# hrdkjain/GenIcoNet

Measured on AMD Instinct MI355X. Metric: meshes/sec training throughput, ico2ico I5 batch=36, higher is better.
Workload: dtype f32; 1 GPU; ico2ico AE training, I5, batch 36 per GPU (BASELINE configs[1]); per_gpu_batch=36, global_batch=36, subdivisions=5, parallelism=dp1

## Files before the change

geniconet_amd/csrc/icn_api.cpp:

```cpp
#include <hip/hip_runtime.h>

#include <algorithm>
#include <cmath>
#include <cstdio>
#include <cstdlib>
#include <cstring>
#include <map>
#include <mutex>
#include <stdexcept>
#include <string>
#include <tuple>
#include <vector>

#include "../../include/icn_ext.h"
#include "../../include/icn_curvature.h"
#include "../../include/icn_gauss.h"
#include "../../include/icn_measure.h"
#include "icn_geometry.h"
#include "icn_launch.h"
#include "icn_streamk.h"

namespace {

thread_local std::string g_err;
// ... 1 lines not shown
int fail(const std::string& msg) {
    g_err = msg;
    return -1;
}

#define ICN_HIP(expr)                                                                       \
    do {                                                                                    \
        hipError_t e_ = (expr);                                                             \
        if (e_ != hipSuccess) throw std::runtime_error(std::string(#expr) + ": " + hipGetErrorString(e_)); \
    } while (0)

template <typename R, typename F>
R returns(F&& body) {
    try {
        return body();
    } catch (const std::exception& e) {
        return (R)fail(e.what());
    }
}
template <typename R, typename F>
R returns_or_zero(F&& body) {
    try {
        return body();
    } catch (const std::exception&) {
        return 0;
    }
}
template <typename F>
int guarded(F&& body) {
    return returns<int>([&] { body(); return 0; });
}
template <typename F>
int launched(F&& body) {
    return returns<int>([&] { body(); ICN_HIP(hipGetLastError()); return 0; });
}

template <typename T>
long copy_out(T* dst, size_t cap, const std::vector<T>& v) {
    if (dst) std::memcpy(dst, v.data(), std::min(cap, v.size()) * sizeof(T));
    return (long)v.size();
}

thread_local bool g_dry_run = false;
thread_local size_t g_dry_elems = 0;

template <typename T>
T* upload(const std::vector<T>& v) {
    T* d = nullptr;
    if (v.empty()) return d;
    if (g_dry_run) {
        g_dry_elems += v.size();
        return d;
    }
    ICN_HIP(hipMalloc(reinterpret_cast<void**>(&d), v.size() * sizeof(T)));
    ICN_HIP(hipMemcpy(d, v.data(), v.size() * sizeof(T), hipMemcpyHostToDevice));
    return d;
}

struct DevDma {
    int32_t* code = nullptr;
    int32_t* slots = nullptr;
    int n_slots = 0, E = 1;
};
DevDma upload_dma(const std::vector<int32_t>& idx, int E, int P) {
    icn::DmaTable h;
    icn::build_dma_table(idx, E, P, h);
    DevDma d;
    d.code = upload(h.code);
    d.slots = upload(h.slots);
    d.n_slots = h.n_slots;
    d.E = E;
    return d;
}
struct ConvTables {
    int Pin = 0, Pout = 0, n_in = 0, n_out = 0, E = 1;
    int32_t* fwd = nullptr;
    int32_t* bwd = nullptr;
    int32_t* bwd1 = nullptr;
    int nv = 0, nvp = 0;
    int32_t* vidx = nullptr;
    int32_t* vorder = nullptr;
    uint32_t* vmask32 = nullptr;
    int32_t* vq = nullptr;
    int32_t* perm = nullptr;
    int32_t* bwd_perm = nullptr;
    uint32_t* mask32 = nullptr;
    std::vector<uint32_t> mask32_h;
    int key = 0;
    DevDma d_fwd, d_bwd, d_bwd1, d_virt, d_bwdp;
    int32_t* w7_rows = nullptr;
    uint16_t* w7_pos = nullptr;
    int w7_U = 0;
};
struct UpTables {
    int Pc = 0, Pf = 0, Wf = 0, Wb = 0;
    int32_t *idx_f = nullptr, *idx_b = nullptr;
    float *coef_f = nullptr, *coef_b = nullptr;
};

struct UpconvDev {
    int Pc = 0, Pf = 0, n_slots = 0, E = 1, nseg = 0;
    int seg_cnt[icn::UPCONV_MAX_SEG] = {}, seg_off[icn::UPCONV_MAX_SEG] = {};
    uint32_t seg_mask[icn::UPCONV_MAX_SEG] = {};
    int32_t *pix = nullptr, *code = nullptr, *slot_idx = nullptr;
    float *alpha = nullptr, *slot_coef = nullptr;
};

struct EllSplitDev {
    int W = 0, n_ovf = 0, W_ovf = 0;
    int32_t *idx = nullptr, *ovf_rows = nullptr, *ovf_idx = nullptr;
    float *coef = nullptr, *ovf_coef = nullptr;
};
EllSplitDev upload_ell_split(const icn::Ell& e, int W_main) {
    EllSplitDev d;
    const int W = e.width;
    d.W = W_main;
    d.W_ovf = std::max(W - W_main, 0);
    std::vector<int32_t> idx((size_t)e.rows * W_main, icn::IDX_ZERO), ovf_rows, ovf_idx;
    std::vector<float> coef((size_t)e.rows * W_main, 0.f), ovf_coef;
    for (int r = 0; r < e.rows; ++r) {
        for (int k = 0; k < std::min(W, W_main); ++k) {
            idx[(size_t)r * W_main + k] = e.idx[(size_t)r * W + k];
            coef[(size_t)r * W_main + k] = e.coef[(size_t)r * W + k];
        }
        if (W > W_main && e.idx[(size_t)r * W + W_main] != icn::IDX_ZERO) {
            ovf_rows.push_back(r);
            for (int k = W_main; k < W; ++k) {
                ovf_idx.push_back(e.idx[(size_t)r * W + k]);
                ovf_coef.push_back(e.coef[(size_t)r * W + k]);
            }
        }
    }
    d.n_ovf = (int)ovf_rows.size();
    d.idx = upload(idx);
    d.coef = upload(coef);
    d.ovf_rows = upload(ovf_rows);
    d.ovf_idx = upload(ovf_idx);
    d.ovf_coef = upload(ovf_coef);
    return d;
}

struct PatchHost { std::vector<int32_t> prow; std::vector<uint16_t> plocal; int npatch = 0, umax = 0, gridW = 0; };
bool build_patches(const std::vector<int32_t>& idx, int width_in, int width, int H, int W, int ph, int pw, PatchHost& out) {
    out = PatchHost{};
    if (H % ph != 0 || W % pw != 0 || (long)H * W * width_in != (long)idx.size()) return false;
    const int pr_n = H / ph, pc_n = W / pw;
    out.npatch = pr_n * pc_n;
    out.gridW = W;
    out.plocal.assign((size_t)H * W * width, 0xFFFFu);
    std::vector<std::vector<int32_t>> lists(out.npatch);
    for (int p = 0; p < out.npatch; ++p) {
        std::vector<int32_t>& u = lists[p];
        for (int i = 0; i < ph; ++i)
            for (int j = 0; j < pw; ++j) {
                const size_t r = (size_t)((p / pc_n) * ph + i) * W + (p % pc_n) * pw + j;
                for (int k = 0; k < width; ++k) {
                    const int32_t v = idx[r * width_in + k];
                    if (v >= 0) u.push_back(v);
                }
            }
        std::sort(u.begin(), u.end());
        u.erase(std::unique(u.begin(), u.end()), u.end());
        out.umax = std::max(out.umax, (int)u.size());
    }
    out.umax = (out.umax + 31) / 32 * 32;
    if (out.umax == 0 || out.umax >= 0xFFFF) return false;
// ... 7 lines not shown
                for (int k = 0; k < width; ++k) {
                    const int32_t v = idx[r * width_in + k];
                    if (v >= 0) out.plocal[r * width + k] = (uint16_t)(std::lower_bound(u.begin(), u.end(), v) - u.begin());
                }
            }
    }
    return true;
}
struct PatchDev { int32_t* prow = nullptr; uint16_t* plocal = nullptr; int npatch = 0, umax = 0, gridW = 0; };
PatchDev upload_patches(const PatchHost& h) {
    PatchDev d;
    if (getenv("ICN_VERBOSE")) fprintf(stderr, "icn: patch table: %d patches, %d rows per list, grid width %d\n", h.npatch, h.umax, h.gridW);
    d.prow = upload(h.prow);
    d.plocal = upload(h.plocal);
    d.npatch = h.npatch; d.umax = h.umax; d.gridW = h.gridW;
    return d;
}

struct UpconvBwdDev {
    int Pc = 0, Pf = 0;
    PatchDev sc_patch, ga_patch;
    EllSplitDev gather, scatter;
    int32_t* iota = nullptr;
    int32_t* px_srcs = nullptr;
    int32_t* px_cls = nullptr;
    float* cls_coef = nullptr;
    int n_cls = 0;
};

std::mutex g_mu;
std::map<std::tuple<int, int, int>, UpconvDev> g_upconv;
std::map<std::tuple<int, int, int>, UpconvBwdDev> g_upconv_bwd;
std::map<std::tuple<int, int, int, int>, ConvTables> g_conv;
std::map<std::tuple<int, int, int>, UpTables> g_up;

static int wgrad7_union_rows(int stride) {
    if (stride != 1) return 112;
    static const int u1 = [] {
        const char* e = getenv("ICN_W7_U");
        return e ? atoi(e) : 64;
    }();
    if (u1 != 56 && u1 != 64)
        throw std::invalid_argument("icn: ICN_W7_U must be 56 or 64 (the instantiations of k_wgrad7 at stride 1), got " + std::to_string(u1));
    return u1;
}

ConvTables make_conv_tables(int r_in, int stride, int mode) {
    ConvTables t;
    t.n_in = 1 << r_in;
    t.n_out = t.n_in / stride;
    t.Pin = icn::pixels(r_in);
    t.Pout = 10 * t.n_out * t.n_out;
    std::vector<int32_t> fwd, bwd, perm;
    std::vector<uint8_t> mask;
    icn::build_conv_fwd(r_in, stride, mode, fwd);
    t.E = icn::build_conv_bwd(r_in, stride, mode, bwd);
    t.fwd = upload(fwd);
    t.bwd = upload(bwd);
    t.d_fwd = upload_dma(fwd, 1, t.Pout);
    t.d_bwd = upload_dma(bwd, t.E, t.Pin);
    {
        icn::DmaTable h;
        icn::build_dma_table(fwd, 1, t.Pout, h);
        icn::Wg7Table w7;
        if (icn::build_wgrad7(h, t.Pout, wgrad7_union_rows(stride), w7)) {
            t.w7_rows = upload(w7.urow);
            t.w7_pos = upload(w7.upos);
            t.w7_U = w7.U;
        }
    }
    std::vector<int32_t> primary;
    icn::VirtualRows vr;
    icn::split_conv_bwd(r_in, stride, bwd, t.E, primary, vr);
    t.bwd1 = upload(primary);
    t.d_bwd1 = upload_dma(primary, 1, t.Pin);
    t.nv = vr.nv;
    if (vr.nv > 0) {
        std::vector<int32_t> order, vidx_o;
        std::vector<uint8_t> vmask;
        icn::build_virtual_order(vr, t.nvp, order, vidx_o, vmask);
        t.vidx = upload(vidx_o);
        t.vorder = upload(order);
        t.vmask32 = upload(std::vector<uint32_t>(vmask.begin(), vmask.end()));
        t.d_virt = upload_dma(vidx_o, 1, t.nvp);
        t.vq = upload(vr.vq);
    }
    if (stride == 2) {
        icn::build_bwd_row_order(r_in, stride, bwd, t.E, perm, mask);
        t.perm = upload(perm);
        t.mask32_h.assign(mask.begin(), mask.end());
        t.mask32 = upload(t.mask32_h);
        t.key = 1 + ((r_in << 8) | (stride << 4) | mode);
        std::vector<int32_t> bwd_p(bwd.size());
        for (int te = 0; te < icn::NTAPS * t.E; ++te)
            for (int k = 0; k < t.Pin; ++k) bwd_p[(size_t)te * t.Pin + k] = bwd[(size_t)te * t.Pin + perm[k]];
        t.bwd_perm = upload(bwd_p);
        t.d_bwdp = upload_dma(bwd_p, t.E, t.Pin);
    }
    return t;
}
const ConvTables& conv_tables(int r_in, int stride, int mode) {
    int dev = 0;
    ICN_HIP(hipGetDevice(&dev));
    std::lock_guard<std::mutex> lk(g_mu);
    auto key = std::make_tuple(dev, r_in, stride, mode);
    auto it = g_conv.find(key);
    if (it != g_conv.end()) return it->second;
    return g_conv.emplace(key, make_conv_tables(r_in, stride, mode)).first->second;
}

std::map<std::pair<int, int>, int32_t*> g_vf;

const int32_t* vertex_faces(int r) {
    int dev = 0;
    ICN_HIP(hipGetDevice(&dev));
    std::lock_guard<std::mutex> lk(g_mu);
    auto key = std::make_pair(dev, r);
    auto it = g_vf.find(key);
    if (it != g_vf.end()) return it->second;
    std::vector<int32_t> vf;
    icn::build_vertex_faces(r, vf);
    return g_vf.emplace(key, upload(vf)).first->second;
}

std::map<std::pair<int, int>, int32_t*> g_vs;

const int32_t* vertex_stencils(int r) {
    int dev = 0;
    ICN_HIP(hipGetDevice(&dev));
    std::lock_guard<std::mutex> lk(g_mu);
    auto key = std::make_pair(dev, r);
    auto it = g_vs.find(key);
    if (it != g_vs.end()) return it->second;
    std::vector<int32_t> vs;
    icn::build_vertex_stencils(r, vs);
    return g_vs.emplace(key, upload(vs)).first->second;
}

UpTables make_up_tables(int r_in, int mode) {
    icn::Ell f, b;
    icn::build_upsample(r_in, mode, f, b);
    UpTables t;
    t.Pc = b.rows;
    t.Pf = f.rows;
    t.Wf = f.width;
    t.Wb = b.width;
    t.idx_f = upload(f.idx);
    t.coef_f = upload(f.coef);
    t.idx_b = upload(b.idx);
    t.coef_b = upload(b.coef);
    return t;
}
const UpTables& up_tables(int r_in, int mode) {
    int dev = 0;
    ICN_HIP(hipGetDevice(&dev));
    std::lock_guard<std::mutex> lk(g_mu);
    auto key = std::make_tuple(dev, r_in, mode);
    auto it = g_up.find(key);
    if (it != g_up.end()) return it->second;
    return g_up.emplace(key, make_up_tables(r_in, mode)).first->second;
}

UpconvDev make_upconv_tables(int r_in, int mode) {
    icn::UpconvTable h;
    icn::build_upconv_fwd(r_in, mode, h);
    UpconvDev d;
    d.Pc = h.Pc; d.Pf = h.Pf; d.n_slots = h.n_slots; d.E = h.E; d.nseg = h.nseg;
    for (int i = 0; i < h.nseg; ++i) { d.seg_cnt[i] = h.seg_cnt[i]; d.seg_off[i] = h.seg_off[i]; d.seg_mask[i] = h.seg_mask[i]; }
// ... 227 lines not shown
    a.wt = bn ? static_cast<const float*>(p.packed_b3) : wreg;
}
size_t conv_ws_bytes(int op, int B, int Cin, int C0, int C1, int r_in, int stride) {
    const int C = C0 + C1, n_out = (1 << r_in) / stride, M = B * 10 * n_out * n_out;
    const size_t wbytes = wpack_bytes((size_t)7 * Cin * C);
    switch (op) {
        case ICN_OP_CONV_FWD:
            if (!icn::gather_gemm_supported(Cin, C)) return 0;
            return wbytes + (C1 ? align256((size_t)C * sizeof(float)) : 0) +
                   align256((size_t)B * table_counts(r_in, stride).slots_fwd * Cin * sizeof(float)) + sk_ws_bytes();
        case ICN_OP_CONV_BWD_DATA: {
            if (!icn::gather_gemm_supported(C, Cin)) return 0;
            const TableCounts c = table_counts(r_in, stride);
            return wbytes + align256((size_t)B * c.nv * Cin * sizeof(float)) +
                   (C1 ? 2 : 1) * align256((size_t)B * c.slots_bwd * C0 * sizeof(float)) + sk_ws_bytes();
        }
        case ICN_OP_CONV_BWD_WEIGHT:
            return wgrad_partial_bytes(M, Cin, C, C0) + wgrad_bias_partial_bytes(M, Cin, C, C0) +
                   align256((size_t)B * table_counts(r_in, stride).slots_fwd * Cin * sizeof(float));
        default: return 0;
    }
}

char* at(void* ws, size_t off) { return static_cast<char*>(ws) + off; }

void conv_fwd_impl(const float* x, const float* w0, const float* b0, const float* w1, const float* b1, float* y0, float* y1, int B,
                   int Cin, int C0, int C1, int r_in, int stride, const ConvTables& t, void* ws, hipStream_t s) {
    const int C = C0 + C1;
    const size_t wbytes = wpack_bytes((size_t)7 * Cin * C);
    float* wf = static_cast<float*>(ws);
    float* bias_cat = (w1 && b0) ? reinterpret_cast<float*>(at(ws, wbytes)) : nullptr;
    const size_t side_off = wbytes + (w1 ? align256((size_t)C * sizeof(float)) : 0);
    float* side = reinterpret_cast<float*>(at(ws, side_off));
    int* sk_flag = reinterpret_cast<int*>(at(ws, side_off + align256((size_t)B * table_counts(r_in, stride).slots_fwd * Cin * sizeof(float))));
    float* sk_part = reinterpret_cast<float*>(reinterpret_cast<char*>(sk_flag) + align256((size_t)icn::CONV_SK_FLAGS * sizeof(int)));
    icn::PrologueArgs p{};
    p.zero = sk_flag; p.n_zero = icn::CONV_SK_FLAGS;
    p.w = w0; p.w2 = w1; p.packed = wf; p.Cout = C0; p.Cout2 = C1; p.Cin = Cin; p.transpose = 0;
    p.bias = b0; p.bias2 = b1; p.bias_cat = bias_cat;
    p.src = x; p.slots = t.d_fwd.slots; p.side = side; p.n_slots = t.d_fwd.n_slots; p.E = 1; p.B = B; p.Ps = t.Pin; p.K = Cin;
    p.ns = t.n_in;
    icn::GatherGemmArgs a{};
    a.src = x; a.bias = w1 ? bias_cat : b0; a.dst = y0; a.dst2 = w1 ? y1 : nullptr; a.N0 = C0;
    a.idx = t.fwd; a.dcode = t.d_fwd.code; a.side = side; a.n_slots = t.d_fwd.n_slots;
    a.M = B * t.Pout; a.Ps = t.Pin; a.Pd = t.Pout; a.K = Cin; a.N = C; a.E = 1; a.ns = t.n_in;
    a.algo_flops = 2.0 * 7 * Cin * C * (double)B * t.Pout;
    a.sk_part = sk_part; a.sk_flag = sk_flag;
    choose_arith(a, p, wf, (size_t)7 * Cin * C, false);
    icn::launch_conv_prologue(p, s);
    icn::launch_gather_gemm_auto(a, s);
}

void conv_bwd_data_impl(const float* dy0, const float* dy1, const float* w0, const float* w1, float* dx, int B, int Cin, int C0,
                        int C1, int r_in, int stride, const ConvTables& t, void* ws, hipStream_t s) {
    const int C = C0 + C1;
    const size_t wbytes = wpack_bytes((size_t)7 * Cin * C);
    const TableCounts tc = table_counts(r_in, stride);
    const size_t side_bytes = align256((size_t)B * tc.slots_bwd * C0 * sizeof(float));
    float* wb = static_cast<float*>(ws);
    float* vout = reinterpret_cast<float*>(at(ws, wbytes));
    float* side = reinterpret_cast<float*>(at(ws, wbytes + align256((size_t)B * tc.nv * Cin * sizeof(float))));
    float* side2 = dy1 ? reinterpret_cast<float*>(reinterpret_cast<char*>(side) + side_bytes) : nullptr;
    int* sk_flag = reinterpret_cast<int*>(reinterpret_cast<char*>(side) + (dy1 ? 2 : 1) * side_bytes);
    float* sk_part = reinterpret_cast<float*>(reinterpret_cast<char*>(sk_flag) + align256((size_t)icn::CONV_SK_FLAGS * sizeof(int)));
    const bool split = stride == 1 && t.nv > 0 && t.nv * 8 < t.Pin;
    const DevDma& dm = split ? t.d_bwd1 : (stride == 2 ? t.d_bwdp : t.d_bwd);
    const DevDma& ds = split ? t.d_virt : dm;
    icn::PrologueArgs p{};
    p.w = w0; p.w2 = w1; p.packed = wb; p.Cout = C0; p.Cout2 = C1; p.Cin = Cin; p.transpose = 1;
    p.src = dy0; p.src2 = dy1; p.slots = ds.slots; p.side = side; p.side2 = side2; p.n_slots = ds.n_slots; p.E = ds.E; p.B = B;
    p.Ps = t.Pout; p.K = C0; p.ns = t.n_out;
    p.zero = sk_flag; p.n_zero = icn::CONV_SK_FLAGS;
    icn::GatherGemmArgs a{};
    a.src = dy0; a.src2 = dy1; a.dst = dx; a.N0 = Cin;
    a.idx = split ? t.bwd1 : (stride == 2 ? t.bwd_perm : t.bwd); a.dcode = dm.code; a.side = side; a.side2 = side2;
    a.n_slots = dm.n_slots; a.perm = t.perm; a.mask32 = t.mask32;
    a.mask32_host = t.mask32_h.empty() ? nullptr : t.mask32_h.data(); a.mask_key = t.key;
    a.M = B * t.Pin; a.Ps = t.Pout; a.Pd = t.Pin; a.K = C; a.N = Cin; a.E = split ? 1 : t.E; a.ns = t.n_out;
    a.algo_flops = 2.0 * 7 * Cin * C * (double)B * t.Pout;
    a.sk_part = sk_part; a.sk_flag = sk_flag;
    choose_arith(a, p, wb, (size_t)7 * Cin * C, split);
    icn::launch_conv_prologue(p, s);
    icn::launch_gather_gemm_auto(a, s);
    if (split) {
        icn::GatherGemmArgs v = a;
        v.wt = wb; v.arith_bn = 0;
        v.sk_part = nullptr; v.sk_flag = nullptr;
        v.dst = vout; v.idx = t.vidx; v.dcode = t.d_virt.code; v.n_slots = t.d_virt.n_slots; v.perm = t.vorder; v.mask32 = t.vmask32;
        v.M = B * t.nvp; v.Pd = t.nvp; v.E = 1;
        v.algo_flops = 0.0;
        icn::launch_gather_gemm_auto(v, s);
        icn::launch_row_scatter_add(vout, dx, t.vq, B, t.nv, t.nvp, t.Pin, Cin, s);
    }
}

void conv_bwd_weight_impl(const float* x, const float* dy0, const float* dy1, float* dw0, float* db0, float* dw1, float* db1, int B,
                          int Cin, int C0, int C1, const ConvTables& t, void* ws, hipStream_t s) {
    const int C = C0 + C1, M = B * t.Pout;
    float* partial = static_cast<float*>(ws);
    float* bpart = (db0 || db1) ? reinterpret_cast<float*>(at(ws, wgrad_partial_bytes(M, Cin, C, C0))) : nullptr;
    float* side = reinterpret_cast<float*>(at(ws, wgrad_partial_bytes(M, Cin, C, C0) + wgrad_bias_partial_bytes(M, Cin, C, C0)));
    const bool mfma = icn::wgrad_supported(Cin, C);
    if (mfma) {
        icn::PrologueArgs p{};
        p.Cin = Cin; p.src = x; p.slots = t.d_fwd.slots; p.side = side; p.n_slots = t.d_fwd.n_slots; p.E = 1; p.B = B; p.Ps = t.Pin;
        p.K = Cin; p.ns = t.n_in;
        icn::launch_conv_prologue(p, s);
    }
    icn::WgradArgs a{};
    a.x = x; a.dy = dy0; a.dy2 = dy1; a.Cout0 = C0; a.idx = t.fwd; a.dcode = mfma ? t.d_fwd.code : nullptr; a.side = side;
    a.n_slots = t.d_fwd.n_slots; a.partial = partial; a.bias_partial = bpart; a.dw = dw0; a.dbias = db0; a.dw2 = dw1; a.dbias2 = db1;
    a.M = M; a.Ps = t.Pin; a.Pd = t.Pout; a.Cin = Cin; a.Cout = C; a.ns = t.n_in;
    a.algo_flops = 2.0 * 7 * Cin * C * (double)M;
    a.w7_rows = t.w7_rows; a.w7_pos = t.w7_pos; a.w7_U = t.w7_U;
    icn::launch_wgrad(a, s);
}

}

namespace icn {
const char* const PROF_NAMES[PROF_KINDS] = {"k_conv_dma<128, 128, false>", "k_conv_dma<128, 64, false>", "k_conv_dma<64, 128, false>",
                                            "k_conv_dma<64, 64, false>",
                                            "k_gather_gemm<128, 128>", "k_gather_gemm<128, 64>", "k_gather_gemm<64, 128>",
                                            "k_gather_gemm<64, 64>", "k_wgrad_dma<128, 128>", "k_wgrad_dma<128, 64>",
                                            "k_wgrad_dma<64, 128>", "k_wgrad_dma<64, 64>", "k_wgrad<128, 128>", "k_wgrad<128, 64>",
                                            "k_wgrad<64, 128>", "k_wgrad<64, 64>", "k_conv_dma<128, 128, true>",
                                            "k_conv_dma<128, 64, true>", "k_conv_dma<64, 128, true>", "k_conv_dma<64, 64, true>",
                                            "k_conv_dma_sk<64, 128, false>", "k_conv_dma_sk<64, 64, false>", "k_conv_dma_sk<64, 128, true>",
                                            "k_conv_dma_sk<64, 64, true>", "k_wgrad7",
                                            "k_conv_dma8<64, 128, false>", "k_conv_dma8<64, 128, true>", "k_conv_dma_sk8<64, 128, false>",
                                            "k_conv_dma_sk8<64, 128, true>", "k_conv_dense_sk<64, 128>", "k_conv_dense_sk<64, 64>", "k_conv_single_sk<64, 128>",
                                            "k_conv_single_sk<64, 64>", "k_wgrad_dense<128, 128>", "k_wgrad_dense<128, 64>",
                                            "k_wgrad_dense<64, 128>", "k_wgrad_dense<64, 64>",
                                            "k_conv_b3_sk<128, 128, 8>", "k_conv_b3_sk<128, 64, 4>", "k_conv_b3_dense_sk<128, 128, 8>",
                                            "k_conv_b3_dense_sk<128, 64, 4>", "k_wgrad7<.., 1>", "k_wgrad_dma<.., 1>", "k_wgrad_dense<.., 1>", "k_conv_b3<128, BN, NW>",
                                            "k_conv_b3_single_sk<128, 128, 8>", "k_conv_b3_single_sk<128, 64, 4>",
                                            "k_point_to_mesh", "k_point_to_mesh_bwd_point", "k_point_to_mesh_bwd_vertex",
                                            "k_p2m_grid_bounds", "k_p2m_grid_count", "k_p2m_grid_scan", "k_p2m_grid_fill",
                                            "k_p2m_grid_query",
                                            "k_msample_area", "k_msample_scan", "k_msample_point", "k_msample_bwd_record",
                                            "k_msample_bwd_vertex",
                                            "k_fnormal_agree", "k_fnormal_agree_bwd_record",
                                            "k_fnormal_agree_bwd_vertex",
                                            "k_mesh_measure_face", "k_mesh_measure_finish", "k_mesh_measure_bwd",
                                            "k_mesh_cotlap_fwd", "k_mesh_willmore_finish", "k_mesh_willmore_upstream", "k_mesh_cotlap_bwd",
                                            "k_mesh_angle_defect_fwd", "k_mesh_angle_defect_bwd"};
void prof_mark_begin(int kind, double flops, hipStream_t s) {
    if (!g_prof_on) return;
    g_prof_mu.lock();
    if (!g_prof_on || g_prof_used >= g_prof.size() || (g_prof_only >= 0 && kind != g_prof_only)) { g_prof_mu.unlock(); return; }
    ProfRec& r = g_prof[g_prof_used];
    r.kind = kind;
    r.flops = flops;
    (void)hipEventRecord(r.e0, s);
    g_prof_open = true;
}
void prof_mark_end(hipStream_t s) {
    if (!g_prof_open) return;
    (void)hipEventRecord(g_prof[g_prof_used].e1, s);
    ++g_prof_used;
    g_prof_open = false;
    g_prof_mu.unlock();
}
}

extern "C" {

// ... 1013 lines not shown
```

geniconet_amd/csrc/icn_geometry.cpp:

```cpp
#include "icn_geometry.h"

#include <algorithm>
#include <cstdlib>
#include <array>
#include <cmath>
#include <map>
#include <stdexcept>

namespace icn {

const int TAP_DA[NTAPS] = {0, 1, 0, -1, -1, 0, 1};
const int TAP_DB[NTAPS] = {0, 0, 1, 1, 0, -1, -1};

namespace {

struct Pt {
    int c, a, b;
};

inline Pt prev1(int, Pt p) { return {(p.c + 4) % 5, p.a + p.b, -p.a}; }
inline Pt prev2(int n, Pt p) { return {(p.c + 4) % 5, p.a + n, p.b - n}; }
inline Pt prev3(int n, Pt p) { return {(p.c + 4) % 5, 3 * n - p.b, p.a + p.b - n}; }
inline Pt next1(int, Pt p) { return {(p.c + 1) % 5, -p.b, p.a + p.b}; }
inline Pt next2(int n, Pt p) { return {(p.c + 1) % 5, p.a - n, p.b + n}; }
// ... 70 lines not shown
            if (q >= 0)
                lists[(size_t)t * Pin + q].push_back(p);
            else if (q <= IDX_POLE)
                pole_src[IDX_POLE - q].push_back(p);
        }
        for (int k = 0; k < 2; ++k) {
            if (pole_src[k].empty()) continue;
            std::vector<int32_t> want;
            for (int c = 0; c < 5; ++c) want.push_back(corner_pixel(no, k, c));
            std::sort(want.begin(), want.end());
            std::sort(pole_src[k].begin(), pole_src[k].end());
            if (want != pole_src[k]) throw std::logic_error("icn: pole taps are not the corner pixels");
            for (int c = 0; c < 5; ++c) lists[(size_t)t * Pin + corner_pixel(n, k, c)].push_back(IDX_POLE - k);
        }
    }
    size_t E = 1;
    for (auto& l : lists) E = std::max(E, l.size());
    out.assign((size_t)NTAPS * E * Pin, IDX_ZERO);
    for (int t = 0; t < NTAPS; ++t)
        for (int q = 0; q < Pin; ++q) {
            auto& l = lists[(size_t)t * Pin + q];
            std::stable_sort(l.begin(), l.end(), [](int32_t x, int32_t y) { return (x >= 0) > (y >= 0); });
            for (size_t e = 0; e < l.size(); ++e) out[((size_t)t * E + e) * Pin + q] = l[e];
        }
    return (int)E;
}

void split_conv_bwd(int r_in, int stride, const std::vector<int32_t>& bwd_idx, int E, std::vector<int32_t>& primary,
                    VirtualRows& vr) {
    const int n = 1 << r_in, Pin = 10 * n * n;
    (void)stride;
    primary.assign((size_t)NTAPS * Pin, IDX_ZERO);
    std::vector<std::array<int32_t, NTAPS>> rows;
    vr = VirtualRows{};
    for (int q = 0; q < Pin; ++q) {
        std::array<std::vector<int32_t>, NTAPS> leftover;
        size_t levels = 0;
        for (int t = 0; t < NTAPS; ++t) {
            bool have_primary = false;
            for (int e = 0; e < E; ++e) {
                const int32_t v = bwd_idx[((size_t)t * E + e) * Pin + q];
                if (v == IDX_ZERO) continue;
                if (v >= 0 && !have_primary) {
                    primary[(size_t)t * Pin + q] = v;
                    have_primary = true;
                } else {
                    leftover[t].push_back(v);
                }
            }
            levels = std::max(levels, leftover[t].size());
        }
        for (size_t l = 0; l < levels; ++l) {
            std::array<int32_t, NTAPS> row;
            for (int t = 0; t < NTAPS; ++t) row[t] = l < leftover[t].size() ? leftover[t][l] : IDX_ZERO;
            rows.push_back(row);
            vr.vq.push_back(q);
        }
    }
    vr.nv = (int)rows.size();
    vr.vidx.assign((size_t)NTAPS * std::max(vr.nv, 1), IDX_ZERO);
    for (int v = 0; v < vr.nv; ++v)
        for (int t = 0; t < NTAPS; ++t) vr.vidx[(size_t)t * vr.nv + v] = rows[v][t];
}

void build_virtual_order(const VirtualRows& vr, int& nvp, std::vector<int32_t>& order, std::vector<int32_t>& vidx_o,
                         std::vector<uint8_t>& mask32) {
    const int nv = vr.nv;
    nvp = (nv + 31) / 32 * 32;
    std::vector<unsigned> taps(nv, 0);
    for (int v = 0; v < nv; ++v)
        for (int t = 0; t < NTAPS; ++t)
            if (vr.vidx[(size_t)t * nv + v] != IDX_ZERO) taps[v] |= 1u << t;
    order.resize(nvp);
    for (int k = 0; k < nvp; ++k) order[k] = k;
    std::stable_sort(order.begin(), order.begin() + nv, [&](int x, int y) { return taps[x] < taps[y]; });
    vidx_o.assign((size_t)NTAPS * nvp, IDX_ZERO);
    mask32.assign(nvp / 32, 0);
    for (int k = 0; k < nv; ++k) {
        for (int t = 0; t < NTAPS; ++t) vidx_o[(size_t)t * nvp + k] = vr.vidx[(size_t)t * nv + order[k]];
        mask32[k / 32] |= (uint8_t)taps[order[k]];
    }
}

void build_dma_table(const std::vector<int32_t>& idx, int E, int P, DmaTable& out) {
    out.E = E;
    out.n_slots = 0;
    out.code.assign((size_t)NTAPS * P, IDX_ZERO);
    out.slots.clear();
    std::map<std::vector<int32_t>, int> slot_of;
    std::vector<int32_t> ent;
    for (int t = 0; t < NTAPS; ++t)
        for (int p = 0; p < P; ++p) {
            ent.clear();
            for (int e = 0; e < E; ++e) {
                const int32_t c = idx[((size_t)t * E + e) * P + p];
                if (c != IDX_ZERO) ent.push_back(c);
            }
            int32_t code = IDX_ZERO;
            if (ent.size() == 1 && ent[0] >= 0) {
                code = ent[0];
            } else if (!ent.empty()) {
                ent.resize(E, IDX_ZERO);
                auto it = slot_of.find(ent);
                if (it == slot_of.end()) {
                    it = slot_of.emplace(ent, out.n_slots++).first;
                    out.slots.insert(out.slots.end(), ent.begin(), ent.end());
                }
                code = -2 - it->second;
            }
            out.code[(size_t)t * P + p] = code;
        }
}

bool build_wgrad7(const DmaTable& d, int P, int max_U, Wg7Table& out) {
    out = Wg7Table{};
    if (P <= 0 || P % WG7_PX != 0 || (size_t)NTAPS * P != d.code.size()) return false;
    const int np = P / WG7_PX;
    std::vector<std::vector<int32_t>> lists(np);
    size_t longest = 0;
    for (int q = 0; q < np; ++q) {
        std::vector<int32_t>& l = lists[q];
        for (int k = 0; k < WG7_PX; ++k)
            for (int t = 0; t < NTAPS; ++t) {
                const int32_t c = d.code[(size_t)t * P + q * WG7_PX + k];
                if (c != IDX_ZERO) l.push_back(c);
            }
        std::sort(l.begin(), l.end(), [](int32_t a, int32_t b) { return (a < 0) != (b < 0) ? b < 0 : (a < 0 ? a > b : a < b); });
        l.erase(std::unique(l.begin(), l.end()), l.end());
        longest = std::max(longest, l.size());
    }
    const int U = max_U;
    if ((int)longest + 1 > U || U % 4 != 0 || (size_t)(U - 1) * WG7_ROW_BYTES > 0xFFFFu) return false;
    out.U = U;
    out.npatch = np;
    out.urow.assign((size_t)np * U, IDX_ZERO);
    out.upos.assign((size_t)np * WG7_PX * 8, (uint16_t)((U - 1) * WG7_ROW_BYTES));
    for (int q = 0; q < np; ++q) {
        const std::vector<int32_t>& l = lists[q];
        for (size_t u = 0; u < l.size(); ++u) out.urow[(size_t)q * U + u] = l[u];
        for (int k = 0; k < WG7_PX; ++k)
            for (int t = 0; t < NTAPS; ++t) {
                const int32_t c = d.code[(size_t)t * P + q * WG7_PX + k];
                if (c == IDX_ZERO) continue;
                const size_t u = std::find(l.begin(), l.end(), c) - l.begin();
                out.upos[((size_t)q * WG7_PX + k) * 8 + t] = (uint16_t)(u * WG7_ROW_BYTES);
            }
    }
    return true;
}

void build_upsample(int r_in, int corner_mode, Ell& fwd, Ell& bwd) {
    check_args(r_in, 1, corner_mode);
    const int n = 1 << r_in, nf = 2 * n;
    const int Pc = 10 * n * n, Pf = 10 * nf * nf;
    std::vector<std::vector<std::pair<int32_t, float>>> rows(Pf), cols(Pc);
    auto add = [&](int q, int32_t v, float w) {
        if (v >= 0) {
            rows[q].push_back({v, w});
        } else if (corner_mode == CORNER_AVERAGE) {
            const int k = v == NORTH ? 0 : 1;
            for (int c = 0; c < 5; ++c) rows[q].push_back({corner_pixel(n, k, c), w * 0.2f});
        }
    };
    for (int c = 0; c < 5; ++c)
        for (int I = 0; I < nf; ++I)
            for (int J = 0; J < 2 * nf; ++J) {
// ... 351 lines not shown
```

geniconet_amd/csrc/icn_geometry.h:

```cpp
#pragma once
#include <cstdint>
#include <vector>

namespace icn {

enum CornerMode { CORNER_ZEROS = 0, CORNER_AVERAGE = 1 };

constexpr int32_t IDX_ZERO = -1;
constexpr int32_t IDX_POLE = -2;

constexpr int NTAPS = 7;
extern const int TAP_DA[NTAPS];
extern const int TAP_DB[NTAPS];

inline int pixels(int r) { return 10 << (2 * r); }

void build_conv_fwd(int r_in, int stride, int corner_mode, std::vector<int32_t>& out);

int build_conv_bwd(int r_in, int stride, int corner_mode, std::vector<int32_t>& out);

struct VirtualRows {
    int nv = 0;
    std::vector<int32_t> vidx;
    std::vector<int32_t> vq;
};
void split_conv_bwd(int r_in, int stride, const std::vector<int32_t>& bwd_idx, int E, std::vector<int32_t>& primary,
                    VirtualRows& vr);

void build_virtual_order(const VirtualRows& vr, int& nvp, std::vector<int32_t>& order, std::vector<int32_t>& vidx_o,
                         std::vector<uint8_t>& mask32);

struct DmaTable {
    int n_slots = 0, E = 1;
    std::vector<int32_t> code;
    std::vector<int32_t> slots;
};
void build_dma_table(const std::vector<int32_t>& idx, int E, int P, DmaTable& out);

constexpr int WG7_PX = 16;
constexpr int WG7_ROW_BYTES = 256;
struct Wg7Table {
    int U = 0, npatch = 0;
    std::vector<int32_t> urow;
    std::vector<uint16_t> upos;
};
bool build_wgrad7(const DmaTable& d, int P, int max_U, Wg7Table& out);

struct Ell {
    int rows = 0, width = 0;
    std::vector<int32_t> idx;
    std::vector<float> coef;
};
void build_upsample(int r_in, int corner_mode, Ell& fwd, Ell& bwd);
void build_upsample_pairs(int r_in, std::vector<int32_t>& out);

constexpr int UPCONV_REGULAR = 19;
constexpr int UPCONV_TAPS = UPCONV_REGULAR + NTAPS;
constexpr int UPCONV_MAX_SEG = 5;
struct UpconvTable {
    int Pc = 0, Pf = 0;
    std::vector<float> alpha;
    int nseg = 0;
    int seg_cnt[UPCONV_MAX_SEG] = {};
    int seg_off[UPCONV_MAX_SEG] = {};
    uint32_t seg_mask[UPCONV_MAX_SEG] = {};
    std::vector<int32_t> pix;
    std::vector<int32_t> code;
    int n_slots = 0, E = 1;
    std::vector<int32_t> slot_idx;
    std::vector<float> slot_coef;
};
void build_upconv_fwd(int r_in, int corner_mode, UpconvTable& out);

void build_upconv_bwd(int r_in, int corner_mode, Ell& out);
void build_upconv_scatter(int r_in, int corner_mode, Ell& out);

void build_bwd_row_order(int r_in, int stride, const std::vector<int32_t>& bwd_idx, int E,
                         std::vector<int32_t>& perm, std::vector<uint8_t>& mask32);

void build_faces(int r, std::vector<int32_t>& faces);

void build_vertex_faces(int r, std::vector<int32_t>& vf);

void build_vertex_stencils(int r, std::vector<int32_t>& vs);

}
```

geniconet_amd/csrc/icn_kernels.hip:

```cpp
#include <hip/hip_runtime.h>
#include <stdint.h>

#include <algorithm>
#include <cfloat>
#include <atomic>
#include <cstdio>
#include <cstdlib>
#include <cstring>
#include <map>
#include <mutex>
#include <tuple>
#include <vector>
#include <stdexcept>
#include <type_traits>
#include <utility>

#include "icn_launch.h"
#include "icn_streamk.h"

#ifndef ICN_CHAIN_PRIO
#define ICN_CHAIN_PRIO 0
#endif
#if ICN_CHAIN_PRIO > 0
#define ICN_CHAIN_SETPRIO() __builtin_amdgcn_s_setprio(ICN_CHAIN_PRIO)
// ... 3009 lines not shown
    }
}

void launch_upconv_gather_px(const float* dy0, const float* dy1, float* g, const int32_t* srcs, const int32_t* cls,
                             const float* cls_coef, int ncls, int B, int Pin, int Pc, int C0, int C1, hipStream_t s) {
    if (ncls < 1 || ncls > UG_CLS_MAX) throw std::invalid_argument("icn: coefficient classes of the per-pixel aggregate out of range");
    const size_t total = (size_t)B * Pc * ((C0 + C1) / 4);
    hipLaunchKernelGGL(k_upconv_gather_px, dim3(xcd_grid(total, 16384)), dim3(256), 0, s, dy0, dy1, g, srcs, cls, cls_coef, ncls,
                       B, Pin, Pc, C0, C1);
}

void launch_upconv_gather(const float* dy0, const float* dy1, float* g, const int32_t* idx, const float* coef, const int32_t* rows,
                          int B, int Pin, int nrows, int rows_total, int C0, int C1, int W, int acc, hipStream_t s) {
    if (nrows <= 0) return;
    const size_t total = (size_t)B * nrows * ((C0 + C1) / 4);
    hipLaunchKernelGGL(k_upconv_gather, dim3((unsigned)std::min((size_t)16384, (total + 255) / 256)), dim3(256), 0, s, dy0, dy1, g, idx,
                       coef, rows, B, Pin, nrows, rows_total, C0, C1, W, acc);
}

void launch_spmm_ell(const float* in, float* out, const int32_t* idx, const float* coef, int B, int Pin, int Pout, int C,
                     int W, hipStream_t s) {
    const int vec = (C % 4 == 0) ? 4 : 1;
    const size_t total = (size_t)B * Pout * (C / vec);
    const int blocks = (int)std::min((size_t)8192, (total + 255) / 256);
    if (vec == 4)
        hipLaunchKernelGGL(k_spmm_ell<4>, dim3(blocks), dim3(256), 0, s, in, out, idx, coef, B, Pin, Pout, C, W);
    else
        hipLaunchKernelGGL(k_spmm_ell<1>, dim3(blocks), dim3(256), 0, s, in, out, idx, coef, B, Pin, Pout, C, W);
}

__global__ void k_conv_generic(const float* __restrict__ src, const float* __restrict__ w, const float* __restrict__ bias,
                               float* __restrict__ dst, const int32_t* __restrict__ idx, int B, int Ps, int Pd, int K, int N,
                               int E, int ns, int transpose) {
    const size_t total = (size_t)B * Pd * N;
    for (size_t i = (size_t)blockIdx.x * blockDim.x + threadIdx.x; i < total; i += (size_t)gridDim.x * blockDim.x) {
        const int n = (int)(i % N);
        const size_t bp = i / N;
        const int p = (int)(bp % Pd), b = (int)(bp / Pd);
        float s = bias ? bias[n] : 0.f;
        for (int t = 0; t < 7; ++t)
            for (int e = 0; e < E; ++e) {
                const int32_t code = idx[((size_t)t * E + e) * Pd + p];
                if (code == -1) continue;
                for (int k = 0; k < K; ++k) {
                    const float wv = transpose ? w[((size_t)k * N + n) * 7 + t] : w[((size_t)n * K + k) * 7 + t];
                    s += gather1(src, code, b, Ps, ns, K, k) * wv;
                }
            }
        dst[i] = s;
    }
}

void launch_conv_generic(const float* src, const float* w, const float* bias, float* dst, const int32_t* idx, int B, int Ps,
                         int Pd, int K, int N, int E, int ns, int transpose, hipStream_t s) {
    const size_t total = (size_t)B * Pd * N;
    const int blocks = (int)std::min((size_t)16384, (total + 255) / 256);
    hipLaunchKernelGGL(k_conv_generic, dim3(blocks), dim3(256), 0, s, src, w, bias, dst, idx, B, Ps, Pd, K, N, E, ns,
                       transpose);
}

__global__ void k_row_scatter_add(const float* __restrict__ src, float* __restrict__ dst, const int32_t* __restrict__ q, int B,
                                  int nv, int nvp, int P, int C) {
    const int c4n = C / 4;
    const size_t total = (size_t)B * nv * c4n;
    for (size_t i = (size_t)blockIdx.x * blockDim.x + threadIdx.x; i < total; i += (size_t)gridDim.x * blockDim.x) {
        const int c = (int)(i % c4n) * 4;
        const size_t bv = i / c4n;
        const int v = (int)(bv % nv), b = (int)(bv / nv);
        const int32_t qv = q[v];
        if (v > 0 && q[v - 1] == qv) continue;
        float* d = dst + ((size_t)b * P + qv) * C + c;
        f32x4 acc = ld4(d);
        for (int k = v; k < nv && q[k] == qv; ++k) acc += ld4(src + ((size_t)b * nvp + k) * C + c);
        *reinterpret_cast<f32x4*>(d) = acc;
    }
}

void launch_row_scatter_add(const float* src, float* dst, const int32_t* q, int B, int nv, int nvp, int P, int C, hipStream_t s) {
    const size_t total = (size_t)B * nv * (C / 4);
    hipLaunchKernelGGL(k_row_scatter_add, dim3((unsigned)std::min((size_t)4096, (total + 255) / 256)), dim3(256), 0, s, src, dst, q, B,
                       nv, nvp, P, C);
}

__global__ __launch_bounds__(256) void k_upconv_prologue(UpconvPrologueArgs a, int npack) {
    if ((int)blockIdx.x < npack) {
        const int Ct = a.Cout + a.Cout2, total = a.NV * Ct * a.Cin;
        for (int i = blockIdx.x * 256 + threadIdx.x; i < total; i += npack * 256) {
            const int ci = i % a.Cin, co = (i / a.Cin) % Ct, v = i / (a.Cin * Ct);
            const float* wp = co < a.Cout ? a.w + ((size_t)co * a.Cin + ci) * 7 : a.w2 + ((size_t)(co - a.Cout) * a.Cin + ci) * 7;
            float acc = 0.f;
#pragma unroll
            for (int t = 0; t < 7; ++t) acc += a.alpha[v * 7 + t] * wp[t];
            a.packed[i] = acc;
        }
        if (a.bias_cat && blockIdx.x == 0)
            for (int c = threadIdx.x; c < Ct; c += 256) a.bias_cat[c] = c < a.Cout ? a.bias[c] : a.bias2[c - a.Cout];
        return;
    }
    const int j = blockIdx.x - npack;
    const int b = j / a.n_slots, sl = j % a.n_slots;
    for (int ch = 4 * threadIdx.x; ch < a.Cin; ch += 4 * 256) {
        f32x4 v = {0.f, 0.f, 0.f, 0.f};
        for (int e = 0; e < a.E; ++e) {
            const int32_t c = a.slot_idx[sl * a.E + e];
            if (c >= 0) v += a.slot_coef[sl * a.E + e] * ld4(a.src + ((size_t)b * a.Ps + c) * a.Cin + ch);
        }
        *reinterpret_cast<f32x4*>(a.side + ((size_t)b * a.n_slots + sl) * a.Cin + ch) = v;
    }
}

void launch_upconv_prologue(const UpconvPrologueArgs& a, hipStream_t s) {
    const int npack = std::min(4096, (a.NV * (a.Cout + a.Cout2) * a.Cin + 255) / 256);
    const int nside = (a.side && a.n_slots > 0) ? a.B * a.n_slots : 0;
    hipLaunchKernelGGL(k_upconv_prologue, dim3(npack + nside), dim3(256), 0, s, a, npack);
}

void launch_conv_prologue(const PrologueArgs& a, hipStream_t s) {
    if (a.packed_b3 && a.b3_bn != 64 && a.b3_bn != 128) throw std::invalid_argument("icn: bf16 weight image needs a column tile of 64 or 128");
    const int npack = (a.w && (a.packed || a.packed_b3)) ? std::min(2048, ((a.Cout + a.Cout2) * a.Cin * 7 + 255) / 256) : 0;
    const int nside = (a.side && a.n_slots > 0) ? a.B * a.n_slots * (a.src2 ? 2 : 1) : 0;
    if (npack + nside == 0 && !a.zero) return;
    hipLaunchKernelGGL(k_conv_prologue, dim3(std::max(1, npack + nside)), dim3(256), 0, s, a, npack);
}

}
```

geniconet_amd/csrc/icn_launch.h:

```cpp
#pragma once
#include <hip/hip_runtime.h>
#include <stdint.h>

namespace icn {

constexpr int MAX_SEGS = 5;
struct RowSegs {
    int nseg;
    int B;
    int row0[MAX_SEGS], cnt[MAX_SEGS], off[MAX_SEGS];
    unsigned mask[MAX_SEGS];
};

struct GatherGemmArgs {
    const float* src;
    const float* src2;
    const float* wt;
    const float* bias;
    float* dst;
    float* dst2;
    int N0;
    const int32_t* idx;
    const int32_t* dcode;
    const float* side;
// ... 10 lines not shown
    float* sk_part;
    int* sk_flag;
    int arith_bn;
};
int arith_mode();
int set_arith_mode(int mode);
unsigned build_flags();
int conv_b3_bn(const GatherGemmArgs& a);
constexpr int CONV_SK_ERROR = 1024;
constexpr int CONV_SK_FLAGS = 1032;
void set_trace_buffer(void* p, size_t n_u64);
int* device_status_word();
int device_status(int clear);
size_t conv_sk_part_bytes();
const int* sk_speed_factors(int occ);
}
#include <vector>
namespace icn {
void build_tile_lists(const uint32_t* mask32_host, int M, int Pd, int bm, int ntn, int ntiles, int grid, int occ, std::vector<int>& h);


struct WgradArgs {
    const float* x;
    const float* dy;
    const float* dy2;
    int Cout0;
    const int32_t* idx;
    const int32_t* dcode;
    const float* side;
    int n_slots;
    float* partial;
    float* bias_partial;
    float* dw;
    float* dbias;
    float* dw2;
    float* dbias2;
    int M, Ps, Pd, Cin, Cout, ns;
    double algo_flops;
    int y_taps;
    int identity_rows;
    const int32_t* w7_rows;
    const uint16_t* w7_pos;
    int w7_U;
};

bool gather_gemm_supported(int K, int N);
bool conv_dma_usable(const GatherGemmArgs& a);
void launch_gather_gemm_auto(const GatherGemmArgs& a, hipStream_t s);

bool wgrad_supported(int Cin, int Cout);
bool wgrad_pair_supported(int M, int Ps, int Pd, int Cin, int Cout0, int Cout1);
int wgrad_splits(int M, int Cin, int Cout, int Cout0 = 0);
int wgrad7_splits(int M, int Pd, int Cin, int Cout, int Cout0);
void launch_wgrad(const WgradArgs& a, hipStream_t s);
bool stem_supported(int Cin, int Cout);
void launch_stem_fwd(const float* x, const float* w, const float* bias, float* y, const int32_t* idx, int M, int Ps, int Pd,
                     int Cin, int Cout, int ns, hipStream_t s);

void launch_upconv_gather(const float* dy0, const float* dy1, float* g, const int32_t* idx, const float* coef, const int32_t* rows,
                          int B, int Pin, int nrows, int rows_total, int C0, int C1, int W, int acc, hipStream_t s);

struct PatchTab { const int32_t* prow; const uint16_t* plocal; int npatch, umax, gridW; };
bool upconv_patch_usable(const PatchTab& t, int B, size_t rows_per_sample, int C0, int C1);
void launch_upconv_scatter_lds(const float* z, const float* bias, float* y0, float* y1, const PatchTab& t, const float* coef, int B,
                               int zrows, int Pout, int C0, int C1, hipStream_t s);
void launch_upconv_gather_lds(const float* dy0, const float* dy1, float* g, const PatchTab& t, const int32_t* cls,
                              const float* cls_coef, int ncls, int B, int Pin, int Pc, int C0, int C1, hipStream_t s);

constexpr int UPCONV_PX_CLASSES = 32;
void launch_upconv_gather_px(const float* dy0, const float* dy1, float* g, const int32_t* srcs, const int32_t* cls,
                             const float* cls_coef, int ncls, int B, int Pin, int Pc, int C0, int C1, hipStream_t s);

void launch_upconv_scatter(const float* z, const float* bias, float* y0, float* y1, const int32_t* idx, const float* coef,
                           const int32_t* rows, int B, int zrows, int nrows, int Pout, int C0, int C1, int W, int acc, hipStream_t s);

void launch_spmm_ell(const float* in, float* out, const int32_t* idx, const float* coef, int B, int Pin, int Pout, int C,
                     int W, hipStream_t s);

void launch_conv_generic(const float* src, const float* w, const float* bias, float* dst, const int32_t* idx, int B, int Ps,
                         int Pd, int K, int N, int E, int ns, int transpose, hipStream_t s);

void launch_row_scatter_add(const float* src, float* dst, const int32_t* q, int B, int nv, int nvp, int P, int C, hipStream_t s);

struct PrologueArgs {
    const float* w; const float* w2; float* packed; int Cout, Cout2, Cin, transpose;
    const float* bias; const float* bias2; float* bias_cat;
    const float* src; const float* src2; const int32_t* slots; float* side; float* side2; int n_slots, E, B, Ps, K, ns;
    int* zero; int n_zero;
    int b3_flat_n;
    void* packed_b3; int b3_bn;
};
void launch_conv_prologue(const PrologueArgs& a, hipStream_t s);

struct UpconvPrologueArgs {
    const float* w; const float* w2; float* packed; int Cout, Cout2, Cin, NV; const float* alpha;
    const float* bias; const float* bias2; float* bias_cat;
    const float* src; const int32_t* slot_idx; const float* slot_coef; float* side; int n_slots, E, B, Ps;
};
void launch_upconv_prologue(const UpconvPrologueArgs& a, hipStream_t s);

bool bn_supported(int C);
int bn_chunks(int M);
void launch_bn_stats(const float* x, int M, int C, float eps, float momentum, float* running_mean, float* running_var, float* stat,
                     float* ws, hipStream_t s);
void launch_bn_stats2(const float* a, const float* b, int M, int C, float eps_a, float mom_a, float* rm_a, float* rv_a, float* stat_a,
                      float eps_b, float mom_b, float* rm_b, float* rv_b, float* stat_b, float* ws, hipStream_t s);
void launch_bn_relu_fwd(const float* a, const float* b, const float* stat_a, const float* stat_b, const float* ga, const float* ba,
                        const float* gb, const float* bb, float* y, int M, int C, hipStream_t s);
void launch_bn_relu_bwd(const float* dy, const float* a, const float* b, const float* stat_a, const float* stat_b, const float* ga,
                        const float* ba, const float* gb, const float* bb, float* da, float* db, float* sums, float* ws, int M, int C,
                        float* dbeta_a, float* dgamma_a, float* dbeta_b, float* dgamma_b, hipStream_t s);

bool head_supported(int Cin, int Cout);
int head_chunks(int M);
void launch_head_fwd(const float* x, const float* w, const float* bias, float* y, int M, int Cin, int Cout, hipStream_t s);
void launch_head_bwd(const float* dy, const float* y, const float* x, const float* w, float* dx, float* dw, float* db, float* ws,
                     int M, int Cin, int Cout, hipStream_t s);

int p2p_loss_blocks(int B, int P);
void launch_p2p_loss_fwd(const float* grid, const float* target, const int32_t* vf, float* partial, float* terms, int B, int P, int n,
                         float f_pos, float f_nor, float f_lap, int lap_mode, hipStream_t s);
void launch_p2p_loss_bwd_pos(const float* grid, const float* target, const float* upstream, float f_pos, float* dgrid, int B, int P,
                             int n, hipStream_t s);
void launch_p2p_loss_bwd(const float* grid, const float* target, const int32_t* vf, const float* upstream, float f_pos, float f_nor,
                         float f_lap, int lap_mode, float* dgrid, float* aux, int B, int P, int n, hipStream_t s);
void launch_mesh_reg_fwd(const float* grid, const int32_t* vs, float* partial, float* terms, int B, int P, int n, float f_edge,
                         float f_ncons, float f_smooth, float edge_length, hipStream_t s);
void launch_mesh_reg_bwd(const float* grid, const int32_t* vs, const float* upstream, float f_edge, float f_ncons, float f_smooth,
                         float edge_length, float* dgrid, float* aux, int B, int P, int n, hipStream_t s);

int kld_blocks(size_t n);
void launch_kld_fwd(const float* mu, const float* logvar, size_t n, float* out, float* partial, hipStream_t s);
void launch_kld_bwd(const float* mu, const float* logvar, const float* upstream, size_t n, float* dmu, float* dlogvar, hipStream_t s);
void launch_reparam_fwd(const float* mu, const float* logvar, const float* eps, size_t n, float* z, hipStream_t s);
void launch_reparam_bwd(const float* dz, const float* logvar, const float* eps, size_t n, float* dmu, float* dlogvar, hipStream_t s);

void launch_point_to_mesh(const float* pts, const float* vts, const int32_t* faces, int B, int P, int V, int F, float* dist,
                          int32_t* face, int32_t* kind, hipStream_t s);
void launch_point_to_mesh_bwd(const float* pts, const float* vts, const int32_t* faces, const int32_t* face, const int32_t* kind,
                              const float* ddist, int B, int P, int V, int F, float* dpts, float* dvts, void* ws, hipStream_t s);

int p2m_grid_res(int F);
size_t point_to_mesh_grid_bytes(int B, int F);
hipError_t launch_point_to_mesh_grid(const float* pts, const float* vts, const int32_t* faces, int B, int P, int V, int F, float* dist,
                                     int32_t* face, int32_t* kind, void* ws, hipStream_t s);

size_t mesh_sample_cdf_bytes(int B, int F);
void launch_mesh_sample_fwd(const float* vts, const int32_t* faces, const float* u, int B, int S, int V, int F, float* points,
                            int32_t* face, float* weights, void* ws, hipStream_t s);
void launch_mesh_sample_bwd(const int32_t* faces, const int32_t* face, const float* weights, const float* dpoints, int B, int S, int V,
                            int F, float* dvts, void* ws, hipStream_t s);

size_t vertex_records_bytes(size_t n);
void launch_vertex_scatter(int prof_kind, void* ws, int B, int n, int V, float* dvts, hipStream_t s);

void launch_face_normal_agree_fwd(const float* va, const int32_t* faces_a, const int32_t* face_a, int Va, int Fa, const float* vb,
                                  const int32_t* faces_b, const int32_t* face_b, int Vb, int Fb, int B, int S, int oriented, float* t,
                                  hipStream_t s);
void launch_face_normal_agree_bwd(const float* va, const int32_t* faces_a, const int32_t* face_a, int Va, int Fa, const float* vb,
                                  const int32_t* faces_b, const int32_t* face_b, int Vb, int Fb, int B, int S, int oriented,
                                  const float* dt, float* dva, float* dvb, void* ws, hipStream_t s);

size_t mesh_measure_bytes(int B, int F);
void launch_mesh_measure_fwd(const float* vts, const int32_t* faces, int B, int V, int F, float* area, float* volume, void* ws,
                             hipStream_t s);
void launch_mesh_measure_bwd(const float* vts, const int32_t* faces, const int32_t* offsets, const int32_t* corners, const float* darea,
// ... 51 lines not shown
```

Before: 5902 meshes/s.

## Fuse virtual-row dgrad gather-GEMM and scatter-add into one seam kernel

Replaces the split backward-data path's second gather-GEMM over padded virtual rows plus the row scatter-add with a single MFMA kernel. Each block owns one seam destination row, walks that row's tap/code entries from a new host-built seam table, and accumulates directly into dx. This removes the intermediate vout buffer, one kernel launch and the padded virtual-row compute. In exchange it adds a read-modify-write of dx with no atomics, which is only safe because each block owns a distinct row, and the new path adds channel-count constraints. A debug flag keeps the old path available.

```diff
diff --git a/geniconet_amd/csrc/icn_api.cpp b/geniconet_amd/csrc/icn_api.cpp
--- a/geniconet_amd/csrc/icn_api.cpp
+++ b/geniconet_amd/csrc/icn_api.cpp
@@ -107,6 +107,9 @@
     int32_t* vorder = nullptr;
     uint32_t* vmask32 = nullptr;
     int32_t* vq = nullptr;
+    int seam_nq = 0, seam_n_ent = 0;
+    int32_t* seam_ent = nullptr;
+    int32_t* seam_start = nullptr;
     int32_t* perm = nullptr;
     int32_t* bwd_perm = nullptr;
     uint32_t* mask32 = nullptr;
@@ -280,8 +283,19 @@
         t.vidx = upload(vidx_o);
         t.vorder = upload(order);
         t.vmask32 = upload(std::vector<uint32_t>(vmask.begin(), vmask.end()));
-        t.d_virt = upload_dma(vidx_o, 1, t.nvp);
+        icn::DmaTable hv;
+        icn::build_dma_table(vidx_o, 1, t.nvp, hv);
+        t.d_virt.code = upload(hv.code);
+        t.d_virt.slots = upload(hv.slots);
+        t.d_virt.n_slots = hv.n_slots;
+        t.d_virt.E = 1;
         t.vq = upload(vr.vq);
+        icn::SeamTable st;
+        icn::build_seam_table(vr, order, hv, t.nvp, st);
+        t.seam_nq = st.nq;
+        t.seam_n_ent = st.n_ent;
+        t.seam_ent = upload(st.ent);
+        t.seam_start = upload(st.start);
     }
     if (stride == 2) {
         icn::build_bwd_row_order(r_in, stride, bwd, t.E, perm, mask);
@@ -675,7 +689,10 @@
     choose_arith(a, p, wb, (size_t)7 * Cin * C, split);
     icn::launch_conv_prologue(p, s);
     icn::launch_gather_gemm_auto(a, s);
-    if (split) {
+    if (split && !(icn::debug_flags() & 524288)) {
+        icn::launch_dgrad_seam(dy0, dy1, side, side2, wb, dx, t.seam_ent, t.seam_start, t.seam_nq, B, t.Pout, t.Pin, C0, C, Cin,
+                               t.d_virt.n_slots, s);
+    } else if (split) {
         icn::GatherGemmArgs v = a;
         v.wt = wb; v.arith_bn = 0;
         v.sk_part = nullptr; v.sk_flag = nullptr;
diff --git a/geniconet_amd/csrc/icn_geometry.cpp b/geniconet_amd/csrc/icn_geometry.cpp
--- a/geniconet_amd/csrc/icn_geometry.cpp
+++ b/geniconet_amd/csrc/icn_geometry.cpp
@@ -176,6 +176,29 @@
     }
 }
 
+void build_seam_table(const VirtualRows& vr, const std::vector<int32_t>& order, const DmaTable& virt, int nvp, SeamTable& out) {
+    out = SeamTable{};
+    const int nv = vr.nv;
+    if ((int)order.size() != nvp || virt.code.size() != (size_t)NTAPS * nvp || nvp < nv)
+        throw std::logic_error("icn: seam table: order / DmaTable do not belong to these virtual rows");
+    std::vector<int> row_of(nv, -1);
+    for (int k = 0; k < nv; ++k) row_of[order[k]] = k;
+    for (int v = 0; v < nv; ++v) {
+        if (row_of[v] < 0 || (v > 0 && vr.vq[v] < vr.vq[v - 1])) throw std::logic_error("icn: seam table: virtual rows out of order");
+        if (v == 0 || vr.vq[v] != vr.vq[v - 1]) {
+            out.start.push_back(out.n_ent);
+            ++out.nq;
+        }
+        for (int t = 0; t < NTAPS; ++t) {
+            const int32_t c = virt.code[(size_t)t * nvp + row_of[v]];
+            if (c == IDX_ZERO) continue;
+            out.ent.insert(out.ent.end(), {vr.vq[v], t, c});
+            ++out.n_ent;
+        }
+    }
+    out.start.push_back(out.n_ent);
+}
+
 void build_dma_table(const std::vector<int32_t>& idx, int E, int P, DmaTable& out) {
     out.E = E;
     out.n_slots = 0;
diff --git a/geniconet_amd/csrc/icn_geometry.h b/geniconet_amd/csrc/icn_geometry.h
--- a/geniconet_amd/csrc/icn_geometry.h
+++ b/geniconet_amd/csrc/icn_geometry.h
@@ -29,6 +29,14 @@
 
 void build_virtual_order(const VirtualRows& vr, int& nvp, std::vector<int32_t>& order, std::vector<int32_t>& vidx_o,
                          std::vector<uint8_t>& mask32);
+
+struct SeamTable {
+    int n_ent = 0, nq = 0;
+    std::vector<int32_t> ent;
+    std::vector<int32_t> start;
+};
+struct DmaTable;
+void build_seam_table(const VirtualRows& vr, const std::vector<int32_t>& order, const DmaTable& virt, int nvp, SeamTable& out);
 
 struct DmaTable {
     int n_slots = 0, E = 1;
diff --git a/geniconet_amd/csrc/icn_kernels.hip b/geniconet_amd/csrc/icn_kernels.hip
--- a/geniconet_amd/csrc/icn_kernels.hip
+++ b/geniconet_amd/csrc/icn_kernels.hip
@@ -3115,6 +3115,96 @@
                        nv, nvp, P, C);
 }
 
+constexpr int SEAM_KC = 32;
+constexpr int SEAM_BT = 64;
+constexpr int SEAM_CT = 64;
+
+__global__ __launch_bounds__(256) __attribute__((amdgpu_waves_per_eu(5))) void k_dgrad_seam(const float* __restrict__ dy0, const float* __restrict__ dy1,
+                                                    const float* __restrict__ side, const float* __restrict__ side2,
+                                                    const float* __restrict__ wb, float* __restrict__ dx,
+                                                    const int32_t* __restrict__ ent, const int32_t* __restrict__ start, int B, int bt,
+                                                    int Ps, int Pd, int C0, int C, int Cin, int n_slots) {
+    constexpr int CT = SEAM_CT, NCT = CT / 32, RS = SEAM_KC + 4, WL = CT / 32, DL = SEAM_BT / 32;
+    static_assert(NCT * (SEAM_BT / 32) == 4, "k_dgrad_seam: one (column tile, sample tile) per wave");
+    __shared__ __attribute__((aligned(16))) float wl[CT * RS];
+    __shared__ __attribute__((aligned(16))) float dyl[SEAM_BT * RS];
+    const int tid = threadIdx.x, wv = tid >> 6, l31 = tid & 31, h = (tid >> 5) & 1;
+    const int ct = wv % NCT, st = wv / NCT;
+    const int b0 = blockIdx.y * bt, nb = min(min(bt, SEAM_BT), B - b0), c0 = blockIdx.z * CT;
+    const int e0 = start[blockIdx.x], e1 = start[blockIdx.x + 1];
+    if (e1 <= e0) return;
+    const int q = ent[3 * e0];
+    if (q < 0 || q >= Pd) return;
+    const int nk = C / SEAM_KC, steps = (e1 - e0) * nk;
+    const int srow = tid >> 3, sk4 = tid & 7;
+    f32x16 acc;
+    f32x4 wr[WL], dr[DL];
+#pragma unroll
+    for (int r = 0; r < 16; ++r) acc[r] = 0.f;
+
+    for (int s = -1; s < steps; ++s) {
+        if (s >= 0) {
+            __syncthreads();
+#pragma unroll
+            for (int j = 0; j < WL; ++j) *reinterpret_cast<f32x4*>(&wl[(srow + 32 * j) * RS + 4 * sk4]) = wr[j];
+#pragma unroll
+            for (int j = 0; j < DL; ++j) *reinterpret_cast<f32x4*>(&dyl[(srow + 32 * j) * RS + 4 * sk4]) = dr[j];
+            __syncthreads();
+        }
+        if (s + 1 < steps) {
+            const int e = e0 + (s + 1) / nk, kc = ((s + 1) % nk) * SEAM_KC;
+            const int t = ent[3 * e + 1], code = ent[3 * e + 2];
+            const bool ok = ent[3 * e] == q && t >= 0 && t < 7 && (code >= 0 ? code < Ps : (code <= -2 && -2 - code < n_slots));
+#pragma unroll
+            for (int j = 0; j < WL; ++j)
+                wr[j] = ok ? ld4(wb + ((size_t)t * Cin + c0 + srow + 32 * j) * C + kc + 4 * sk4) : f32x4{0.f, 0.f, 0.f, 0.f};
+            const bool second = kc >= C0;
+            const int Ck = second ? C - C0 : C0, kk = second ? kc - C0 : kc;
+#pragma unroll
+            for (int j = 0; j < DL; ++j) {
+                dr[j] = f32x4{0.f, 0.f, 0.f, 0.f};
+                const int b = srow + 32 * j;
+                if (ok && b < nb) {
+                    const float* row = code >= 0 ? (second ? dy1 : dy0) + ((size_t)(b0 + b) * Ps + code) * Ck
+                                                 : (second ? side2 : side) + ((size_t)(b0 + b) * n_slots + (-2 - code)) * Ck;
+                    dr[j] = ld4(row + kk + 4 * sk4);
+                }
+            }
+        }
+        if (s < 0) continue;
+        if (32 * st >= nb) continue;
+#pragma unroll
+        for (int kq = 0; kq < SEAM_KC / 8; ++kq) {
+            const f32x4 a = *reinterpret_cast<const f32x4*>(&wl[(32 * ct + l31) * RS + 8 * kq + 4 * h]);
+            const f32x4 d = *reinterpret_cast<const f32x4*>(&dyl[(32 * st + l31) * RS + 8 * kq + 4 * h]);
+#pragma unroll
+            for (int m = 0; m < 4; ++m) acc = __builtin_amdgcn_mfma_f32_32x32x2f32(a[m], d[m], acc, 0, 0, 0);
+        }
+    }
+    const int b = 32 * st + l31;
+    if (b < nb) {
+        float* d = dx + ((size_t)(b0 + b) * Pd + q) * Cin + c0 + 32 * ct + 4 * h;
+#pragma unroll
+        for (int g = 0; g < 4; ++g) {
+            const f32x4 v = {acc[4 * g], acc[4 * g + 1], acc[4 * g + 2], acc[4 * g + 3]};
+            *reinterpret_cast<f32x4*>(d + 8 * g) = ld4(d + 8 * g) + v;
+        }
+    }
+}
+
+void launch_dgrad_seam(const float* dy0, const float* dy1, const float* side, const float* side2, const float* wb, float* dx,
+                       const int32_t* ent, const int32_t* start, int nq, int B, int Ps, int Pd, int C0, int C, int Cin, int n_slots,
+                       hipStream_t s) {
+    if (nq <= 0 || B <= 0) return;
+    if (Cin % 64 != 0 || C % SEAM_KC != 0 || C0 % SEAM_KC != 0 || C0 < SEAM_KC || C0 > C || (dy1 == nullptr) != (C0 == C) ||
+        (n_slots > 0 && (side == nullptr || (dy1 != nullptr && side2 == nullptr))))
+        throw std::invalid_argument("icn: seam pass of bwd-data needs Cin % 64 == 0, channel counts in multiples of 32 and a side buffer per dy");
+    const int ntile = (B + SEAM_BT - 1) / SEAM_BT, bt = (B + ntile - 1) / ntile;
+    if (ntile > 65535) throw std::invalid_argument("icn: seam pass of bwd-data: batch too large");
+    hipLaunchKernelGGL(k_dgrad_seam, dim3(nq, ntile, Cin / SEAM_CT), dim3(256), 0, s, dy0, dy1, side, side2, wb, dx, ent, start, B, bt, Ps,
+                       Pd, C0, C, Cin, n_slots);
+}
+
 __global__ __launch_bounds__(256) void k_upconv_prologue(UpconvPrologueArgs a, int npack) {
     if ((int)blockIdx.x < npack) {
         const int Ct = a.Cout + a.Cout2, total = a.NV * Ct * a.Cin;
diff --git a/geniconet_amd/csrc/icn_launch.h b/geniconet_amd/csrc/icn_launch.h
--- a/geniconet_amd/csrc/icn_launch.h
+++ b/geniconet_amd/csrc/icn_launch.h
@@ -116,6 +116,10 @@
 
 void launch_row_scatter_add(const float* src, float* dst, const int32_t* q, int B, int nv, int nvp, int P, int C, hipStream_t s);
 
+void launch_dgrad_seam(const float* dy0, const float* dy1, const float* side, const float* side2, const float* wb, float* dx,
+                       const int32_t* ent, const int32_t* start, int nq, int B, int Ps, int Pd, int C0, int C, int Cin, int n_slots,
+                       hipStream_t s);
+
 struct PrologueArgs {
     const float* w; const float* w2; float* packed; int Cout, Cout2, Cin, transpose;
     const float* bias; const float* bias2; float* bias_cat;
```

After: 5935 meshes/s, median of 6. Within noise of the previous version (+0.6%).
